# rhofield/rho-tts

Measured on AMD Instinct MI355X. Metric: audio-sec/wall-sec (RTF) Qwen3-TTS-1.7B batch=32, higher is better.
Workload: dtype bf16; 1 GPU; Qwen3-TTS-1.7B bf16, batch 32/GPU, 30-s reference clone, 10-word sentences (44 frames each), sampling=top-k 50 T 0.9, seeded synthetic weights; value counts delivered (post-processed) audio; global_batch=32, parallelism=dp1

## Files before the change

rho_tts_amd/csrc/generate.hip:

```cpp
#include "model_internal.h"

using namespace rtm;

namespace {

__global__ void k_frame_inc(int32_t* f) { if (threadIdx.x == 0) *f += 1; }
}

struct rt_gen_run {
    struct Staging { std::vector<int32_t> tid, cid, slot, pos, last, dst; };
    struct Lane {
        int b0 = 0, n = 0;
        hipStream_t stream = nullptr;
        float *xt = nullptr, *hn_f32 = nullptr, *xp = nullptr, *logits = nullptr, *rowsq_t = nullptr, *rowsq_p = nullptr;
        bf16_t *hn = nullptr, *hn_p = nullptr;
        int32_t *d_slot_b = nullptr, *d_pos_b = nullptr, *d_pos_p2 = nullptr, *d_zero_pos = nullptr, *d_frame = nullptr, *d_frame_off = nullptr;
        int64_t* d_items = nullptr;
        uint8_t* d_seen = nullptr;
        DecWs dwt, dwp;
        StackWs wt, wp;
        bool done = false;
    };
    rt_model* m = nullptr;
    rt_ctx* ctx = nullptr;
// ... 375 lines not shown
            ns = 1;
        } else {
            RT_TRY(gemm_rows(m, ln.hn_p + roff * Hp, n, PW(m, "pred.head" + std::to_string(q)), ln.logits, &ns));
        }
        SampleArgs sp{};
        sp.logits = ln.logits; sp.n_slabs = ns; sp.M = n; sp.V = Vp;
        sp.do_sample = A.predictor.do_sample; sp.temperature = A.predictor.temperature; sp.top_k = A.predictor.top_k;
        sp.top_p = A.predictor.top_p; sp.rep_penalty = 1.0f; sp.seen = nullptr; sp.suppress_from = Vp; sp.allow_token = -1;
        sp.seed_ptr = d_seed; sp.item_ids = ln.d_items; sp.frame = 0; sp.group = q + 1;
        sp.forced = d_forced ? d_forced + (size_t)(q + 1) * B + ln.b0 : nullptr; sp.forced_fs = (int64_t)G * B;
        sp.out = codes + q + 1; sp.out_stride = G; sp.out_fs = codes_fs; sp.eos_token = -1; sp.eos_flag = nullptr; sp.eos_fs = 0;
        sp.logits_copy = A.d_trace_predictor ? A.d_trace_predictor + ((size_t)q * B + ln.b0) * Vp : nullptr;
        sp.copy_fs = (int64_t)(G - 1) * B * Vp;
        sp.frame_ptr = ln.d_frame; sp.frame_off = ln.d_frame_off; sp.eos_live = 0; sp.min_frames = 0;
        const bool fuse_emb = col && m->has_mtp() && g_fuse_sample_embed && q < G - 2 && Vp <= 4096 && Hp % 8 == 0;
        if (fuse_emb) {
            sp.emb_table = m->proj_emb[q]; sp.emb_H = Hp; sp.emb_norm_w = m->pred.L[0].ln1; sp.emb_rowsq = ln.rowsq_p; sp.emb_rowsq_n = NTp;
            sp.emb_x_tiled = ln.dwp.xT; sp.emb_a_tiled = ln.dwp.xa;
        }
        RT_TRY(launch_sample(ctx, sp));
        if (q < G - 2) {
            if (fuse_emb) {
            } else if (col && m->has_mtp()) {
                RT_TRY(launch_embed_rowsq(ctx, nullptr, 0, m->proj_emb[q], codes + q + 1, G, ln.d_frame, codes_fs, n, Hp, nullptr, ln.rowsq_p,
                                          NTp, ln.dwp.xT, ln.dwp.xa, m->pred.L[0].ln1));
            } else if (col) {
                RT_TRY(launch_embed_rowsq(ctx, m->d_frame_srcs + q + 1, 1, nullptr, codes + q + 1, G, ln.d_frame, codes_fs, n, Hp, nullptr,
                                          ln.rowsq_p, NTp, ln.dwp.xT, ln.dwp.xa, m->pred.L[0].ln1));
            } else if (m->has_mtp()) RT_TRY(launch_gather_f32(ctx, m->proj_emb[q], Hp, codes + q + 1, n, ln.xp, nullptr, G, ln.d_frame, codes_fs));
            else RT_TRY(launch_gather_sum(ctx, m->d_frame_srcs + q + 1, 1, codes + q + 1, n, H, nullptr, nullptr, nullptr, ln.xp, nullptr, G, ln.d_frame, codes_fs));
            m->prof_class = 2;
            if (col) {
                RT_TRY(stack_decode(m, m->pred, ln.dwp, ln.dwp.xT, ln.rowsq_p, n, ln.d_slot_b, ln.d_zero_pos, q + 2, true, nullptr, ln.b0, true));
            } else {
                RT_TRY(stack_forward(m, m->pred, ln.wp, ln.xp, n, ln.d_slot_b, ln.d_zero_pos, q + 2, ln.hn_p, nullptr));
            }
        }
    }
    m->prof_class = 0;
    return RT_OK;
}

int rt_gen_run::enqueue_b(Lane& ln) {
    const int n = ln.n;
    int32_t* codes = d_codes + (size_t)ln.b0 * G;
    const bool inc_early = col && G <= 16 && g_frame_inc_fold;
    if (col && G <= 16) {
        RT_TRY(launch_embed_rowsq(ctx, m->d_frame_srcs, G, nullptr, codes, G, ln.d_frame, codes_fs, n, H, pad_t, ln.rowsq_t, NTt, ln.dwt.xT,
// ... 275 lines not shown
```

rho_tts_amd/csrc/kernels.h:

```cpp
#pragma once
#include "common.h"
#include "knobs.h"

struct PackedW {
    const bf16_t* data = nullptr;
    int N = 0, K = 0;
    int Np = 0, Kp = 0;
    size_t bytes() const { return (size_t)Np * Kp * 2; }
    const bf16_t* data16 = nullptr;
    int Np16 = 0;
};

struct GemmA {
    const void* ptr = nullptr;
    const void* ptr_lo = nullptr;
    int is_f32 = 0;
    int split = 0;
    int64_t M = 0;
    int Cin = 0;
    int taps = 1;
    int tap_stride = 1;
    int tap_offset = 0;
    int rows_out = 0;
    int rows_in = 0;
// ... 67 lines not shown
int launch_gemm_col(rt_ctx* ctx, const ColArgs& a, const PackedW& w, hipEvent_t ev_start = nullptr, hipEvent_t ev_stop = nullptr);
struct RowsqGather {
    const float* table = nullptr;
    const int32_t* idx = nullptr;
    int idx_stride = 1, first = 0;
    const int32_t* frame_ptr = nullptr;
    int64_t idx_frame_stride = 0;
};
int launch_rowsq(rt_ctx* ctx, const float* x, int M, int H, float* rowsq, int rowsq_n, float* x_tiled = nullptr,
                 bf16_t* a_tiled = nullptr, const float* norm_w = nullptr, const int32_t* src_rows = nullptr,
                 const int32_t* dst_rows = nullptr, const RowsqGather* gather = nullptr);

struct GatherSrc;
int launch_embed_rowsq(rt_ctx* ctx, const GatherSrc* d_srcs, int n_src, const float* f32_table, const int32_t* d_idx, int idx_stride,
                       const int32_t* frame_ptr, int64_t idx_frame_stride, int M, int H, const float* add_vec, float* rowsq, int rowsq_n,
                       float* x_tiled, bf16_t* a_tiled, const float* norm_w, int32_t* frame_inc = nullptr, unsigned* arrive = nullptr);

int launch_norm_tiled_rows(rt_ctx* ctx, const float* x_tiled, const float* rowsq, int rowsq_n, const float* w, float eps, int M, int H,
                           float* out);

int launch_add_rmsnorm(rt_ctx* ctx, float* x, int M, int H, const float* slabs, int n_slabs, const float* slab_bias,
                       const float* scale, const float* w, float eps, bf16_t* out_bf16, float* out_f32);
int launch_silu_mul(rt_ctx* ctx, const float* slabs, int n_slabs, int M, int I, bf16_t* out, float* out_f32 = nullptr);
int launch_reduce_slabs(rt_ctx* ctx, const float* slabs, int n_slabs, int64_t M, int N, const float* bias, int act,
                        float* out_f32, bf16_t* out_bf16);

struct KvCache {
    bf16_t* k = nullptr;
    bf16_t* v = nullptr;
    int layers = 0, slots = 0, kv_heads = 0, max_pos = 0, head_dim = 0;
    bf16_t* k_lo = nullptr;
// ... 66 lines not shown
    int eos_token;
    int32_t* eos_flag;
    float* logits_copy;
    const int32_t* frame_ptr;
    const int32_t* frame_off;
    int64_t out_fs, eos_fs, forced_fs, copy_fs;
    int eos_live, min_frames;
    long long* stamps;
    const float* emb_table;
    int emb_H;
    const float* emb_norm_w;
    float* emb_rowsq;
    int emb_rowsq_n;
    float* emb_x_tiled;
    bf16_t* emb_a_tiled;
};
int launch_sample(rt_ctx* ctx, const SampleArgs& a);


int launch_dwconv_ln(rt_ctx* ctx, const float* x, int B, int T, int C, const float* w , const float* b,
                     const float* ln_w, const float* ln_b, float eps, float* out_f32);
int launch_code_embed_mean(rt_ctx* ctx, const bf16_t* table, int codebook, int Q, int H, const int32_t* codes ,
                           int64_t rows, float* out_f32);

bool launch_final_conv_ok(int C);
int launch_final_conv(rt_ctx* ctx, const bf16_t* hi, const bf16_t* lo, int B, int T, int C, const float* w, const float* bias, float* wav,
                      int64_t wav_stride);
int launch_f32_to_bf16(rt_ctx* ctx, const float* x, int64_t n, bf16_t* out);

int launch_enc_conv0(rt_ctx* ctx, const float* pcm, int64_t T, int C, int k, const float* w , const float* bias, float* x,
// ... 5 lines not shown
```

rho_tts_amd/csrc/knobs.h:

```cpp
#pragma once
#include "common.h"

#define RT_KNOBS(X) \
    X(0, g_skinny_variant, 0, 0, 2, "legacy skinny GEMM: 0 k_gemm_skinny, 1 k_gemm_skinny2<.,4>, 2 k_gemm_skinny2<.,8>") \
    X(100, g_decode_col, 1, 0, 1, "0 legacy 9-launch split-K decode, 1 column-owner GEMM + fused attention (5 launches per layer)") \
    X(200, g_use_graph, 1, 0, 1, "0 eager decode frames, 1 replayed from captured hipGraphs") \
    X(300, g_pred_nt, 0, 0, 1, "predictor weights: 0 cacheable loads (Infinity-Cache resident across its 15 passes), 1 non-temporal") \
    X(400, g_decode_lanes, 1, 1, 8, "decode lanes: groups of items decoding concurrently on their own streams (rt_generate)") \
    X(500, g_col_split, 0, 0, 4, "sub-tile split of narrow decode GEMMs: 0 automatic (col_split_for), 1 / 2 / 4 forced") \
    X(600, g_tile96, 1, 0, 1, "1: 128x96 workgroup tiles for N = 96 / 192 (codec decoder), 0: always 128x128") \
    X(700, g_col_rows64, 1, 0, 1, "1: one 64-row decode GEMM launch for the predictor's two-position pass, 0: two 32-row launches") \
    X(800, g_fuse_sample_embed, 1, 0, 1, "1: sampler + next-input embedding in one launch (predictor groups), 0: separate k_embed_rowsq") \
    X(900, g_prefill_fill, 3, 0, 99, "workgroups per CU a prefill GEMM's split-K aims for") \
    X(1000, g_xcd_order, 1, 0, 1, "1: tiled GEMMs run a row tile's column tiles back to back on one XCD") \
    X(1100, g_final_conv, 1, 0, 1, "the codec decoder's last conv: 1 its own LDS-window kernel, 0 a one-column GEMM") \
    X(1200, g_conv_win, 1, 0, 1, "1: k>1 convs on operand planes keep their input window in LDS (k_conv_win), 0: per-tap kernel") \
    X(1300, g_sync_parts, 0, 0, 1, "1: rt_generate waits for the stream after every frame part (bounds the dispatches in flight; profiling aid)") \
    X(1400, g_eos_check_every, 8, 1, 99, "frames between two host looks at the device-side end-of-sequence flags (1 = every frame)") \
    X(1500, g_attn_mfma, 0, 0, 2, "the talker's shared-prefix decode attention: 0 vector unit, 1 / 2 matrix cores with four rows / one row per workgroup (attention_mfma.hip); 1 measured " \
        "16.6 us per launch against 13.3 us for the vector-unit kernel at batch 32 / 460 prefix rows, so off") \
    X(1600, g_col_split4, 0, 0, 1, "1: the automatic split may go to quarter tiles (N <= 1024 on 256 CUs); measured 1.4 ms/step slower than half tiles") \
    X(1700, g_handover_every, 4, 1, 99, "queued items (n_items > rows): frames between two looks at the flags + row hand-overs.  Measured on the 1.7B model, 512 / 64 ragged texts on 32 " \
        "rows: 2 -> 487 / 445, 3 -> 489 / 445, 4 -> 491 / 447, 6 -> 485 / 445, 8 -> 477 / 428, 12 -> 475 / 434 audio-s/s (a hand-over costs ~1.4 ms, a waiting row 0.13 ms per frame)") \
    X(1800, g_conv_tall, 1, 0, 2, "k>1 convs of the 96- / 192-channel stages: 0 128-row tiles, 1 256-row tiles for long inputs, 2 always") \
    X(1900, g_prefill_mid, 1, 0, 3, "prompt prefills of 65..1024 rows: 0 split-K tiled kernel, 1 k_gemm_mid (no split-K slabs), 2 / 3 force its 64 / 128 tiles") \
    X(2000, g_col_max_rows, 64, 1, 64, "batches up to this many rows decode on the column-owner path.  Above 32 the talker's GEMMs take 64 rows per launch and the predictor's " \
        "two-position first pass runs as two 64-row launches: 715 audio-s/s at batch 64 against 510 at batch 32 (1.7B, bench.py --batch 64) - every weight byte serves twice the rows for " \
        "~1.4x the launch time") \
    X(2100, g_fuse_conv, 1, 0, 1, "1: a 96-channel k>1 conv and the 1x1 conv behind its activation run as one launch (launch_conv_pair); 0 switches the 192-channel pairs off as well") \
    X(2200, g_prefill_attn_mfma, 1, 0, 1, "prompt attention behind a shared voice prefix: 0 vector unit, 1 matrix cores") \
    X(2300, g_col_rows16, 0, 0, 1, "1: decode GEMM launches of <= 16 rows take the 128-VGPR MT = 1 instantiation (two workgroups per CU: decode lanes)") \
    X(2400, g_col_silu_x, 1, 0, 1, "1: gate/up GEMMs whose pairs are 1.5x the CUs run as one round of 1.5-pair workgroups, 0: one pair per workgroup (1.5 rounds)") \
    X(2600, g_conv_unroll, 1, 0, 1, "1: k = 7 convs run the tap-unrolled instantiation of k_conv_win, 0: the generic tap loop") \
    X(2700, g_frame_inc_fold, 0, 0, 1, "1: frame += 1 by the last workgroup of the frame's talker-input launch, 0: k_frame_inc (the fold measured 1-1.8 ms per step SLOWER)") \
    X(2800, g_pair_attn, 1, 0, 1, "1: two-position decode passes append both positions inside the fused attention launch, 0: k_qkv_post + k_attention") \
    X(2900, g_c2w_lean, 1, 0, 1, "1: rt_code2wav drops the third unit's unread residual-stream store and the waveform copy (the last conv writes the caller's buffer)") \
    X(3000, g_fuse_conv192, 1, 0, 1, "1: the 192-channel conv pairs fuse as well, weight fragments staged through LDS")

#define RT_KNOB_ARG(X) \
    X(0, g_skinny_waves_per_cu, 4, 1, 0x7fffffff, "legacy skinny GEMM: split-K is chosen so that about this many waves per CU stream weights")

#define RT_KNOB_EXTERN(base, name, def, lo, hi, doc) extern rt_knob name;
RT_KNOBS(RT_KNOB_EXTERN)
RT_KNOB_ARG(RT_KNOB_EXTERN)
#undef RT_KNOB_EXTERN
extern std::atomic<int> g_tune_epoch;
```

rho_tts_amd/csrc/model_internal.h:

```cpp
#pragma once

#include <algorithm>
#include <chrono>
#include <map>
#include <memory>

#include "kernels.h"


enum SlotKind { K_GEMM = 0, K_TABLE = 1, K_VEC = 2 };

struct Slot {
    std::string name;
    int kind = 0;
    int64_t rows = 0, cols = 0;
    bool set = false;
    PackedW pw;
    bf16_t* tbl = nullptr;
    float* vec = nullptr;
    void* raw = nullptr;
    void* raw16 = nullptr;
};

struct LayerW {
// ... 24 lines not shown
    int64_t last_frames_run = 0, last_rows = 0, last_kept = 0, last_swaps = 0;
    double last_launch_host_us = 0.0;
    rt_ctx* ctx = nullptr;
    rt_model_config cfg{};
    std::vector<Slot> slots;
    std::map<std::string, int> by_name;
    bool finalized = false;
    StackW talker, pred, ctf, etf;
    std::vector<int> enc_ch;
    const float** d_cbT = nullptr;
    std::vector<int> dec_ch;
    float* pad_t = nullptr;
    int pad_t_id = -1;
    float* proj_c0 = nullptr;
    std::vector<float*> proj_emb;
    GatherSrc* d_frame_srcs = nullptr;
    std::vector<float*> exp_vecs;
    std::map<std::string, float*> xvec;
    int prefix_len = 0;
    std::vector<PoolBlock> pool;
    bool prof = false;
    std::vector<std::pair<hipEvent_t, hipEvent_t>> prof_ev;
    size_t prof_used = 0;
    double prof_bytes = 0;
    int prof_class = 0;
    std::vector<std::pair<uint8_t, double>> prof_tag;
    uint64_t graph_sig = 0;
    std::vector<hipGraphExec_t> graphs;
    std::vector<hipStream_t> lane_streams;
    std::vector<hipEvent_t> lane_events;
// ... 44 lines not shown
    bf16_t* act = nullptr;
    float* q = nullptr;
    float* xT = nullptr;
    bf16_t* xa = nullptr;
};
struct TextWs { bf16_t *e = nullptr, *h1 = nullptr; GatherSrc* d_src = nullptr; };
bool prof_events(rt_model* m, double bytes, hipEvent_t* a, hipEvent_t* b);
int gemm_rows(rt_model* m, const bf16_t* A, int rows, const PackedW& W, float* slabs, int* n_slabs);
int gemm_rows_f32(rt_model* m, const float* A, int rows, const PackedW& W, float* slabs, int* n_slabs);
size_t slab_floats(const rt_stack_dims& d, int M, int n_cu = 256);
int alloc_stack_ws(rt_model* m, const rt_stack_dims& d, int M, StackWs* w, bool precise = false);
int stack_forward(rt_model* m, StackW& S, StackWs& w, float* x, int M, const int32_t* row_slot, const int32_t* row_pos, int pos_add,
                  bf16_t* out_bf16, float* out_f32, const int32_t* frame_ptr = nullptr, bool prefix_rows = false);
int alloc_dec_ws(rt_model* m, const rt_stack_dims& d, int M, DecWs* w);
int col_gemm(rt_model* m, const ColArgs& a0, const PackedW& W, bool is_predictor = false);
int stack_decode(rt_model* m, StackW& S, DecWs& w, float* x, float* rowsq, int M, const int32_t* row_slot, const int32_t* row_pos,
                 int pos_add, bool one_row_per_slot = true, const int32_t* frame_ptr = nullptr, int slot_base = -1, bool zero_pos = false);
int col_head(rt_model* m, const bf16_t* xa, const float* rowsq, int rowsq_n, int row_off, int M, int K, float eps,
             const PackedW& W, const float* bias, float* out);
int alloc_text_ws(rt_model* m, int n, TextWs* w);
int text_project(rt_model* m, const int32_t* d_ids, int n, float* out, const TextWs* ws = nullptr);

}
```

rho_tts_amd/csrc/model_load.hip:

```cpp
#include "model_internal.h"

namespace {

__global__ void k_bf16_to_f32(const bf16_t* __restrict__ x, int64_t n, float* __restrict__ out) {
    for (int64_t i = (int64_t)blockIdx.x * blockDim.x + threadIdx.x; i < n; i += (int64_t)gridDim.x * blockDim.x) out[i] = bf16_to_f32(x[i]);
}
__global__ void k_fill_i32(int32_t* p, int n, int v, int step_every, int step) {
    for (int i = blockIdx.x * blockDim.x + threadIdx.x; i < n; i += gridDim.x * blockDim.x) p[i] = v + (step_every > 0 ? (i / step_every) * step : 0);
}
}

namespace rtm {

int pool_get(rt_model* m, size_t bytes, void** out) {
    if (bytes == 0) bytes = 16;
    int best = -1;
    for (size_t i = 0; i < m->pool.size(); ++i)
        if (!m->pool[i].used && m->pool[i].size >= bytes && (best < 0 || m->pool[i].size < m->pool[best].size)) best = (int)i;
    if (best >= 0 && m->pool[best].size <= bytes * 2 + (1 << 20)) {
        m->pool[best].used = true;
        m->pool[best].tag = m->pool_tag;
        *out = m->pool[best].p;
        return RT_OK;
    }
// ... 171 lines not shown
        RT_HIP(m->ctx, hipMemsetAsync(S.kv.v_lo, 0, bytes, m->ctx->stream));
    }
    return RT_OK;
}

int expand_vec(rt_model* m, const float* src, int n, int reps, float** out) {
    float* p = nullptr;
    RT_HIP(m->ctx, hipMalloc((void**)&p, (size_t)n * reps * sizeof(float)));
    for (int r = 0; r < reps; ++r)
        RT_HIP(m->ctx, hipMemcpyAsync(p + (size_t)r * n, src, (size_t)n * sizeof(float), hipMemcpyDeviceToDevice, m->ctx->stream));
    m->exp_vecs.push_back(p);
    *out = p;
    return RT_OK;
}

}

extern "C" {

int rt_model_create(rt_ctx* ctx, const rt_model_config* cfg, rt_model** out_model) {
    if (!ctx || !cfg || !out_model) return rt_fail(ctx, RT_ERR_INVALID, "rt_model_create: null argument");
    *out_model = nullptr;
    const rt_model_config& c = *cfg;
    auto bad_stack = [](const rt_stack_dims& d) {
        return d.hidden < 16 || d.hidden % 16 || d.layers < 1 || d.heads < 1 || d.kv_heads < 1 || d.heads % d.kv_heads ||
               (d.head_dim != 32 && d.head_dim != 64 && d.head_dim != 128) || d.inter % 16 || (d.heads * d.head_dim) % 32 ||
               (d.kv_heads * d.head_dim) % 16;
    };
    if (bad_stack(c.talker) || bad_stack(c.predictor) || bad_stack(c.codec_tf))
        return rt_fail(ctx, RT_ERR_INVALID, "rt_model_create: unsupported stack dimensions (hidden/inter %% 16, head_dim in {32,64,128})");
// ... 29 lines not shown
    for (auto& s : m->slots) { if (s.raw) (void)hipFree(s.raw); if (s.raw16) (void)hipFree(s.raw16); }
    if (m->d_cbT) (void)hipFree((void*)m->d_cbT);
    for (StackW* S : {&m->talker, &m->pred, &m->ctf, &m->etf}) {
        if (S->kv.k) (void)hipFree(S->kv.k);
        if (S->kv.v) (void)hipFree(S->kv.v);
        if (S->kv.k_lo) (void)hipFree(S->kv.k_lo);
        if (S->kv.v_lo) (void)hipFree(S->kv.v_lo);
        if (S->kv.vt_prefix) (void)hipFree(S->kv.vt_prefix);
        if (S->kv.kt_prefix) (void)hipFree(S->kv.kt_prefix);
        if (S->cos) (void)hipFree(S->cos);
        if (S->sin) (void)hipFree(S->sin);
    }
    for (auto& b : m->pool) (void)hipFree(b.p);
    for (auto p : m->exp_vecs) (void)hipFree(p);
    for (auto p : m->proj_emb) (void)hipFree(p);
    if (m->proj_c0) (void)hipFree(m->proj_c0);
    if (m->pad_t) (void)hipFree(m->pad_t);
    if (m->d_frame_srcs) (void)hipFree(m->d_frame_srcs);
    for (auto& e : m->prof_ev) { (void)hipEventDestroy(e.first); (void)hipEventDestroy(e.second); }
    for (auto ex : m->graphs) if (ex) (void)hipGraphExecDestroy(ex);
    for (auto st : m->lane_streams) { (void)hipStreamSynchronize(st); (void)hipStreamDestroy(st); }
    for (auto ev : m->lane_events) (void)hipEventDestroy(ev);
    if (m->fork_event) (void)hipEventDestroy(m->fork_event);
    delete m;
    return RT_OK;
}

int rt_model_tensor_count(rt_model* m) { return m ? (int)m->slots.size() : -1; }

int rt_model_tensor_info(rt_model* m, int32_t index, char* name, size_t name_cap, int64_t* shape2, int32_t* kind) {
// ... 108 lines not shown
    for (int gq = 1; gq < c.n_groups; ++gq) srcs[gq] = {TBL(m, "pred.emb" + std::to_string(gq - 1)), c.talker.hidden};
    RT_HIP(ctx, hipMalloc((void**)&m->d_frame_srcs, sizeof(GatherSrc) * c.n_groups));
    RT_HIP(ctx, hipMemcpy(m->d_frame_srcs, srcs.data(), sizeof(GatherSrc) * c.n_groups, hipMemcpyHostToDevice));
    if (m->has_mtp()) {
        const int Hp = c.predictor.hidden, H = c.talker.hidden;
        auto project = [&](const bf16_t* tbl, int rows, float** out) -> int {
            RT_HIP(ctx, hipMalloc((void**)out, (size_t)rows * Hp * 4));
            GemmA a; a.ptr = tbl; a.M = rows; a.Cin = H;
            GemmEpi e; e.bias = VEC(m, "pred.mtp_b"); e.out_f32 = *out; e.ldc = Hp;
            return launch_gemm(ctx, a, PW(m, "pred.mtp"), e);
        };
        RT_TRY(project(TBL(m, "talker.codec_embedding"), c.codec_vocab, &m->proj_c0));
        m->proj_emb.resize(c.n_groups - 1, nullptr);
        for (int gq = 0; gq < c.n_groups - 1; ++gq) RT_TRY(project(TBL(m, "pred.emb" + std::to_string(gq)), c.predictor_vocab, &m->proj_emb[gq]));
    }
    for (int i = 0; i < c.n_upsample_rates; ++i) {
        const std::string bn = "codec.b" + std::to_string(i);
        for (const char* v : {".u0.a1", ".u0.ib1"}) {
            float* x = nullptr;
            RT_TRY(expand_vec(m, VEC(m, bn + v), m->dec_ch[i + 1], c.upsample_rates[i], &x));
            m->xvec[bn + v] = x;
        }
    }
    RT_HIP(ctx, hipStreamSynchronize(ctx->stream));
    m->finalized = true;
    return RT_OK;
}

int64_t rt_model_weight_bytes(rt_model* m) { return m ? m->weight_bytes : -1; }

// ... 49 lines not shown
```

rho_tts_amd/csrc/model_stack.hip:

```cpp
#include "model_internal.h"

namespace rtm {

bool prof_events(rt_model* m, double bytes, hipEvent_t* a, hipEvent_t* b) {
    *a = *b = nullptr;
    if (!m->prof) return false;
    if (m->prof_used >= m->prof_ev.size()) {
        if (m->prof_ev.size() >= 400000) return false;
        hipEvent_t x, y;
        if (hipEventCreate(&x) != hipSuccess || hipEventCreate(&y) != hipSuccess) return false;
        m->prof_ev.push_back({x, y});
    }
    if (m->prof_tag.size() <= m->prof_used) m->prof_tag.resize(m->prof_used + 1);
    m->prof_tag[m->prof_used] = {(uint8_t)m->prof_class, bytes};
    auto& pr = m->prof_ev[m->prof_used++];
    *a = pr.first;
    *b = pr.second;
    m->prof_bytes += bytes;
    return true;
}

int gemm_rows(rt_model* m, const bf16_t* A, int rows, const PackedW& W, float* slabs, int* n_slabs) {
    if (rows <= 64) {
        const int S = skinny_pick_split(rows, W.N, W.K, m->ctx->n_cu);
// ... 122 lines not shown
    return RT_OK;
}
int col_gemm(rt_model* m, const ColArgs& a0, const PackedW& W, bool is_predictor) {
    const int blk = g_col_rows64 ? 64 : 32;
    for (int r0 = 0; r0 < a0.M; r0 += blk) {
        ColArgs a = a0;
        a.nt = is_predictor ? g_pred_nt.load() : 1;
        a.M = std::min(blk, a0.M - r0);
        a.row_off = a0.row_off + r0;
        hipEvent_t e0, e1;
        prof_events(m, (double)W.N * W.K * 2.0, &e0, &e1);
        RT_TRY(launch_gemm_col(m->ctx, a, W, e0, e1));
    }
    return RT_OK;
}
int stack_decode(rt_model* m, StackW& S, DecWs& w, float* x, float* rowsq, int M, const int32_t* row_slot, const int32_t* row_pos,
                 int pos_add, bool one_row_per_slot, const int32_t* frame_ptr, int slot_base, bool zero_pos) {
    rt_ctx* ctx = m->ctx;
    const rt_stack_dims& d = S.d;
    const int H = d.hidden, sp_h = col_split_for(H, ctx->n_cu), NTh = H / 16 * sp_h, qw = (d.heads + 2 * d.kv_heads) * d.head_dim;
    const bool isp = &S == &m->pred;
    for (int i = 0; i < d.layers; ++i) {
        LayerW& L = S.L[i];
        const float* next_w = (i + 1 < d.layers) ? S.L[i + 1].ln1 : S.norm;
        ColArgs a;
        a.A = w.xa; a.post_scale = 1; a.rowsq = rowsq; a.rowsq_n = NTh; a.eps = d.rms_eps; a.M = M; a.K = H;
        a.epi = COL_STORE; a.out = w.qkv; a.ldc = qw; a.split = col_split_for(qw, ctx->n_cu);
        RT_TRY(col_gemm(m, a, L.wqkv, isp));
        if (one_row_per_slot) {
            RT_TRY(launch_attention_fused(ctx, w.qkv, M, d.heads, d.kv_heads, d.head_dim, L.qn, L.kn, d.rms_eps, S.cos, S.sin, slot_base >= 0 ? nullptr : row_slot,
                                          zero_pos ? nullptr : row_pos, pos_add, S.window, S.kv, i, w.ao, frame_ptr, 1, slot_base));
        } else if (g_pair_attn && M % 2 == 0 && d.heads <= 2 * d.kv_heads && d.heads % d.kv_heads == 0 && row_slot && row_pos) {
            RT_TRY(launch_attention_fused(ctx, w.qkv, M, d.heads, d.kv_heads, d.head_dim, L.qn, L.kn, d.rms_eps, S.cos, S.sin, row_slot, row_pos, pos_add,
                                          S.window, S.kv, i, w.ao, frame_ptr, 1, -1, M / 2));
        } else {
            RT_TRY(launch_qkv_post(ctx, w.qkv, 1, M, d.heads, d.kv_heads, d.head_dim, L.qn, L.kn, d.rms_eps, S.cos, S.sin, row_slot, row_pos,
                                   pos_add, w.q, S.kv, i, frame_ptr));
            RT_TRY(launch_attention(ctx, w.q, M, d.heads, d.kv_heads, d.head_dim, row_slot, row_pos, pos_add, S.window, S.kv, i, w.ao, frame_ptr, 1));
        }
        ColArgs o;
        o.A = w.ao; o.M = M; o.K = d.heads * d.head_dim; o.epi = COL_RESID; o.out = x; o.ldc = H; o.scale = L.ls1;
        o.rowsq_out = rowsq; o.rowsq_out_n = NTh; o.next_bf16 = w.xa; o.next_norm_w = L.ln2; o.split = sp_h;
        RT_TRY(col_gemm(m, o, L.wo, isp));
// ... 47 lines not shown
```

rho_tts_amd/csrc/rowops.hip:

```cpp
#include "kernels.h"

namespace {

typedef __attribute__((ext_vector_type(4))) float f4_t;

__device__ __forceinline__ float block_sum_f32(float v, float* sh) {
    v = wave_sum_f32(v);
    const int w = threadIdx.x >> 6, nw = (blockDim.x + 63) >> 6;
    __syncthreads();
    if ((threadIdx.x & 63) == 0) sh[w] = v;
    __syncthreads();
    float t = 0.f;
    for (int i = 0; i < nw; ++i) t += sh[i];
    return t;
}

__global__ __launch_bounds__(256) void k_add_rmsnorm(float* __restrict__ x, int H, const float* __restrict__ slabs, int n_slabs,
                                                     int64_t slab_stride, const float* __restrict__ slab_bias,
                                                     const float* __restrict__ scale, const float* __restrict__ w, float eps,
                                                     bf16_t* __restrict__ out_bf16, float* __restrict__ out_f32) {
    __shared__ float sh[4];
    constexpr int MAXV = 8;
    const int64_t row = blockIdx.x;
    const int nv = H >> 2;
// ... 132 lines not shown
            uint2 pk;
            pk.x = f32x2_to_bf16x2(wv[0] * v[0], wv[1] * v[1]);
            pk.y = f32x2_to_bf16x2(wv[2] * v[2], wv[3] * v[3]);
            *reinterpret_cast<uint2*>(a_tiled + tile_off((int)row, i * 4, H)) = pk;
        }
    }
    const float tot = block_sum_f32(ss, sh);
    for (int j = threadIdx.x; j < rowsq_n; j += 256) rowsq[row * rowsq_n + j] = j == 0 ? tot : 0.f;
}

__global__ __launch_bounds__(256) void k_embed_rowsq(const GatherSrc* __restrict__ srcs, int n_src, const float* __restrict__ f32_table,
                                                     const int32_t* __restrict__ idx, int idx_stride,
                                                     const int32_t* __restrict__ frame_ptr, int64_t idx_frame_stride, int H,
                                                     const float* __restrict__ add_vec, float* __restrict__ rowsq, int rowsq_n,
                                                     float* __restrict__ x_tiled, bf16_t* __restrict__ a_tiled,
                                                     const float* __restrict__ norm_w, int32_t* frame_inc, unsigned* arrive) {
    constexpr int MAXS = 16;
    __shared__ const bf16_t* sh_tab[MAXS];
    __shared__ float sh[4];
    const int row = blockIdx.x, tid = threadIdx.x;
    if (frame_ptr) idx += (int64_t)(frame_inc ? __atomic_load_n(frame_ptr, __ATOMIC_RELAXED) : *frame_ptr) * idx_frame_stride;
    if (tid < MAXS) {
        const bf16_t* p = nullptr;
        if (tid < n_src) {
            const int id = idx[(int64_t)row * idx_stride + tid];
            if (id >= 0) p = srcs[tid].table + (int64_t)id * srcs[tid].row_stride;
        }
        sh_tab[tid] = p;
    }
    const int fid = f32_table ? idx[(int64_t)row * idx_stride] : -1;
    __syncthreads();
    if (frame_inc && tid == 0 && atomicAdd(arrive, 1u) == gridDim.x - 1) {
        *arrive = 0u;
        atomicAdd(frame_inc, 1);
    }
    float ss = 0.f;
    for (int c = tid * 8; c < H; c += 2048) {
        uint4 raw[MAXS];
#pragma unroll
        for (int j = 0; j < MAXS; ++j) {
            const bf16_t* p = sh_tab[j];
            raw[j] = p ? *reinterpret_cast<const uint4*>(p + c) : uint4{0u, 0u, 0u, 0u};
        }
        float v[8];
#pragma unroll
// ... 15 lines not shown
                }
            }
        }
#pragma unroll
        for (int e = 0; e < 8; ++e) ss += v[e] * v[e];
        const int64_t o = tile_off(row, c, H);
        *reinterpret_cast<f4_t*>(x_tiled + o) = f4_t{v[0], v[1], v[2], v[3]};
        *reinterpret_cast<f4_t*>(x_tiled + o + 4) = f4_t{v[4], v[5], v[6], v[7]};
        const f4_t w0 = *reinterpret_cast<const f4_t*>(norm_w + c), w1 = *reinterpret_cast<const f4_t*>(norm_w + c + 4);
        uint4 pk;
        pk.x = f32x2_to_bf16x2(w0[0] * v[0], w0[1] * v[1]);
        pk.y = f32x2_to_bf16x2(w0[2] * v[2], w0[3] * v[3]);
        pk.z = f32x2_to_bf16x2(w1[0] * v[4], w1[1] * v[5]);
        pk.w = f32x2_to_bf16x2(w1[2] * v[6], w1[3] * v[7]);
        *reinterpret_cast<uint4*>(a_tiled + o) = pk;
    }
    const float tot = block_sum_f32(ss, sh);
    for (int j = tid; j < rowsq_n; j += 256) rowsq[(int64_t)row * rowsq_n + j] = j == 0 ? tot : 0.f;
}

__global__ __launch_bounds__(256) void k_norm_tiled_rows(const float* __restrict__ x_tiled, const float* __restrict__ rowsq, int rowsq_n,
                                                         const float* __restrict__ w, float eps, int H, float* __restrict__ out) {
    __shared__ float sh[4];
    const int row = blockIdx.x;
    float s = 0.f;
    for (int j = threadIdx.x; j < rowsq_n; j += 256) s += rowsq[(int64_t)row * rowsq_n + j];
    const float inv = rsqrtf(block_sum_f32(s, sh) / (float)H + eps);
    for (int c = threadIdx.x * 4; c < H; c += 1024) {
        const f4_t v = *reinterpret_cast<const f4_t*>(x_tiled + tile_off(row, c, H));
        const f4_t wv = *reinterpret_cast<const f4_t*>(w + c);
// ... 251 lines not shown
}

int launch_rowsq(rt_ctx* ctx, const float* x, int M, int H, float* rowsq, int rowsq_n, float* x_tiled, bf16_t* a_tiled,
                 const float* norm_w, const int32_t* src_rows, const int32_t* dst_rows, const RowsqGather* gather) {
    if (M <= 0) return RT_OK;
    const RowsqGather gt = gather ? *gather : RowsqGather{};
    if (gt.table && (src_rows || dst_rows || gt.first < 0 || gt.first > M || !gt.idx))
        return rt_fail(ctx, RT_ERR_INVALID, "rowsq: gathered rows take no row maps (first %d of %d rows)", gt.first, M);
    hipLaunchKernelGGL(k_rowsq, dim3(M), dim3(256), 0, ctx->stream, x, H, rowsq, rowsq_n, x_tiled, a_tiled, norm_w, src_rows, dst_rows, gt);
    RT_HIP(ctx, hipGetLastError());
    return RT_OK;
}

int launch_embed_rowsq(rt_ctx* ctx, const GatherSrc* d_srcs, int n_src, const float* f32_table, const int32_t* d_idx, int idx_stride,
                       const int32_t* frame_ptr, int64_t idx_frame_stride, int M, int H, const float* add_vec, float* rowsq, int rowsq_n,
                       float* x_tiled, bf16_t* a_tiled, const float* norm_w, int32_t* frame_inc, unsigned* arrive) {
    if (M <= 0) return RT_OK;
    if (n_src > 16 || H % 8 || !x_tiled || !a_tiled || !norm_w || !rowsq || rowsq_n < 1 || (n_src > 0 && !d_srcs))
        return rt_fail(ctx, RT_ERR_INVALID, "embed_rowsq: n_src %d (<= 16), H %d (multiple of 8) or a missing buffer", n_src, H);
    if (frame_inc && (f32_table || !arrive || frame_inc != frame_ptr))
        return rt_fail(ctx, RT_ERR_INVALID, "embed_rowsq: the frame counter is advanced by launches over bf16 sources only, with an arrival counter");
    hipLaunchKernelGGL(k_embed_rowsq, dim3(M), dim3(256), 0, ctx->stream, d_srcs, n_src, f32_table, d_idx, idx_stride, frame_ptr,
                       idx_frame_stride, H, add_vec, rowsq, rowsq_n, x_tiled, a_tiled, norm_w, frame_inc, arrive);
    RT_HIP(ctx, hipGetLastError());
    return RT_OK;
}

int launch_norm_tiled_rows(rt_ctx* ctx, const float* x_tiled, const float* rowsq, int rowsq_n, const float* w, float eps, int M, int H,
                           float* out) {
    if (M <= 0) return RT_OK;
    if (H % 8) return rt_fail(ctx, RT_ERR_INVALID, "norm_tiled_rows: H %d not a multiple of 8", H);
    hipLaunchKernelGGL(k_norm_tiled_rows, dim3(M), dim3(256), 0, ctx->stream, x_tiled, rowsq, rowsq_n, w, eps, H, out);
    RT_HIP(ctx, hipGetLastError());
    return RT_OK;
}

int launch_silu_mul(rt_ctx* ctx, const float* slabs, int n_slabs, int M, int I, bf16_t* out, float* out_f32) {
    const int64_t total = (int64_t)M * I / 4;
// ... 88 lines not shown
```

rho_tts_amd/csrc/sampling.hip:

```cpp
#include "kernels.h"

namespace {

__device__ __forceinline__ unsigned mix32(unsigned h) {
    h ^= h >> 16; h *= 0x85EBCA6Bu; h ^= h >> 13; h *= 0xC2B2AE35u; h ^= h >> 16;
    return h;
}
__device__ __forceinline__ float rt_uniform(uint64_t seed, unsigned item, unsigned frame, unsigned group) {
    const unsigned a = mix32((unsigned)(seed & 0xffffffffu) ^ 0x85EBCA6Bu);
    const unsigned b = mix32(a + item * 0x9E3779B1u);
    const unsigned c = mix32(b + frame * 0x85EBCA77u);
    const unsigned d = mix32(c + group * 0xC2B2AE3Du + (unsigned)(seed >> 32));
    return __fmul_rn(__fadd_rn((float)(d >> 8), 0.5f), 1.0f / 16777216.0f);
}
__device__ __forceinline__ unsigned okey(float f) {
    const unsigned u = __float_as_uint(f);
    return (u & 0x80000000u) ? ~u : (u | 0x80000000u);
}

struct Cand { float v; int idx; };
__device__ __forceinline__ bool before(const Cand& a, const Cand& b) { return a.v > b.v || (a.v == b.v && a.idx < b.idx); }

__global__ __launch_bounds__(256) void k_sample(SampleArgs A) {
    extern __shared__ float vals[];
// ... 466 lines not shown
        __syncthreads();
    }
    if (A.stamps && row == 0 && tid == 0) A.stamps[6] = wall_clock64();
    if (tid == 0) {
        if (seen && token >= 0 && token < V) seen[token] = 1;
        int is_eos = 0;
        if (A.eos_token >= 0 && token == A.eos_token) { is_eos = 1; token = 0; }
        if (A.eos_flag) A.eos_flag[row] = is_eos;
        A.out[(int64_t)row * A.out_stride] = token;
        sh_i[0] = token;
    }
    if (A.emb_table) {
        __syncthreads();
        const int tok = sh_i[0];
        const int H = A.emb_H;
        float ss = 0.f;
        if (tid < 256) {
            for (int c = tid * 8; c < H; c += 2048) {
                float e[8];
                const f4s_t a = *reinterpret_cast<const f4s_t*>(A.emb_table + (int64_t)tok * H + c);
                const f4s_t b = *reinterpret_cast<const f4s_t*>(A.emb_table + (int64_t)tok * H + c + 4);
#pragma unroll
                for (int q = 0; q < 4; ++q) { e[q] = 0.f + a[q]; e[4 + q] = 0.f + b[q]; }
#pragma unroll
                for (int q = 0; q < 8; ++q) ss += e[q] * e[q];
                const int64_t o = tile_off(row, c, H);
                *reinterpret_cast<f4s_t*>(A.emb_x_tiled + o) = f4s_t{e[0], e[1], e[2], e[3]};
                *reinterpret_cast<f4s_t*>(A.emb_x_tiled + o + 4) = f4s_t{e[4], e[5], e[6], e[7]};
                const f4s_t w0 = *reinterpret_cast<const f4s_t*>(A.emb_norm_w + c), w1 = *reinterpret_cast<const f4s_t*>(A.emb_norm_w + c + 4);
                uint4 pk;
// ... 10 lines not shown
        __syncthreads();
        const float tot = ((sh_f[0] + sh_f[1]) + sh_f[2]) + sh_f[3];
        for (int j = tid; j < A.emb_rowsq_n; j += NT) A.emb_rowsq[(int64_t)row * A.emb_rowsq_n + j] = j == 0 ? tot : 0.f;
    }
}

}

int launch_sample(rt_ctx* ctx, const SampleArgs& a) {
    if (a.M <= 0) return RT_OK;
    if (a.do_sample && (a.top_k < 1 || a.top_k > 64)) return rt_fail(ctx, RT_ERR_INVALID, "sampling needs 1 <= top_k <= 64 (got %d)", a.top_k);
    if (a.do_sample && !(a.temperature > 0.f)) return rt_fail(ctx, RT_ERR_INVALID, "sampling needs temperature > 0");
    if (a.V > 16384) return rt_fail(ctx, RT_ERR_UNSUPPORTED, "vocabulary %d too large for the sampler", a.V);
    if (a.emb_table && (a.V > 4096 || a.emb_H % 8 || !a.emb_norm_w || !a.emb_rowsq || a.emb_rowsq_n < 1 || !a.emb_x_tiled || !a.emb_a_tiled))
        return rt_fail(ctx, RT_ERR_INVALID, "sample: fused embedding needs V <= 4096, H %% 8 == 0 and all its buffers");
    if (a.V <= 1024) hipLaunchKernelGGL((k_sample_w<4, 4>), dim3(a.M), dim3(256), 0, ctx->stream, a);
    else if (a.V <= 2048) hipLaunchKernelGGL((k_sample_w<4, 8>), dim3(a.M), dim3(512), 0, ctx->stream, a);
    else if (a.V <= 4096) hipLaunchKernelGGL((k_sample_w<4, 16>), dim3(a.M), dim3(1024), 0, ctx->stream, a);
    else hipLaunchKernelGGL(k_sample, dim3(a.M), dim3(256), a.V * sizeof(float), ctx->stream, a);
    RT_HIP(ctx, hipGetLastError());
    return RT_OK;
}
```

Before: 569.7 audio-s/s.

## Precompute predictor layer-0 QKV per code and copy rows instead of GEMM

At model load, the predictor's layer-0 q/k/v projection is precomputed for every code in each codebook group, giving per-group tables of vocab by qkv-width floats. During decode, the kernel that embeds the drawn code (fused sampler or embed_rowsq) also copies that code's qkv row into the workspace, and stack_decode skips the layer-0 QKV GEMM. This removes one GEMM launch and its weight streaming per predictor pass. In exchange it costs extra load time and memory for the tables, adds per-row copy traffic, and the fused sampler path no longer writes the normalized bf16 activations or rowsq, which is safe only if layer 0 never reads them.

```diff
diff --git a/rho_tts_amd/csrc/generate.hip b/rho_tts_amd/csrc/generate.hip
--- a/rho_tts_amd/csrc/generate.hip
+++ b/rho_tts_amd/csrc/generate.hip
@@ -413,24 +413,27 @@
         sp.copy_fs = (int64_t)(G - 1) * B * Vp;
         sp.frame_ptr = ln.d_frame; sp.frame_off = ln.d_frame_off; sp.eos_live = 0; sp.min_frames = 0;
         const bool fuse_emb = col && m->has_mtp() && g_fuse_sample_embed && q < G - 2 && Vp <= 4096 && Hp % 8 == 0;
+        const float* qkv_tab = (col && g_pred_qkv_table && q < G - 2 && q < (int)m->pred_qkv0.size()) ? m->pred_qkv0[q] : nullptr;
+        const int qw_p = (c.predictor.heads + 2 * c.predictor.kv_heads) * c.predictor.head_dim;
         if (fuse_emb) {
             sp.emb_table = m->proj_emb[q]; sp.emb_H = Hp; sp.emb_norm_w = m->pred.L[0].ln1; sp.emb_rowsq = ln.rowsq_p; sp.emb_rowsq_n = NTp;
             sp.emb_x_tiled = ln.dwp.xT; sp.emb_a_tiled = ln.dwp.xa;
+            sp.emb_qkv_table = qkv_tab; sp.emb_qkv_out = ln.dwp.qkv; sp.emb_qkv_n = qw_p;
         }
         RT_TRY(launch_sample(ctx, sp));
         if (q < G - 2) {
             if (fuse_emb) {
             } else if (col && m->has_mtp()) {
                 RT_TRY(launch_embed_rowsq(ctx, nullptr, 0, m->proj_emb[q], codes + q + 1, G, ln.d_frame, codes_fs, n, Hp, nullptr, ln.rowsq_p,
-                                          NTp, ln.dwp.xT, ln.dwp.xa, m->pred.L[0].ln1));
+                                          NTp, ln.dwp.xT, ln.dwp.xa, m->pred.L[0].ln1, nullptr, nullptr, qkv_tab, ln.dwp.qkv, qw_p));
             } else if (col) {
                 RT_TRY(launch_embed_rowsq(ctx, m->d_frame_srcs + q + 1, 1, nullptr, codes + q + 1, G, ln.d_frame, codes_fs, n, Hp, nullptr,
-                                          ln.rowsq_p, NTp, ln.dwp.xT, ln.dwp.xa, m->pred.L[0].ln1));
+                                          ln.rowsq_p, NTp, ln.dwp.xT, ln.dwp.xa, m->pred.L[0].ln1, nullptr, nullptr, qkv_tab, ln.dwp.qkv, qw_p));
             } else if (m->has_mtp()) RT_TRY(launch_gather_f32(ctx, m->proj_emb[q], Hp, codes + q + 1, n, ln.xp, nullptr, G, ln.d_frame, codes_fs));
             else RT_TRY(launch_gather_sum(ctx, m->d_frame_srcs + q + 1, 1, codes + q + 1, n, H, nullptr, nullptr, nullptr, ln.xp, nullptr, G, ln.d_frame, codes_fs));
             m->prof_class = 2;
             if (col) {
-                RT_TRY(stack_decode(m, m->pred, ln.dwp, ln.dwp.xT, ln.rowsq_p, n, ln.d_slot_b, ln.d_zero_pos, q + 2, true, nullptr, ln.b0, true));
+                RT_TRY(stack_decode(m, m->pred, ln.dwp, ln.dwp.xT, ln.rowsq_p, n, ln.d_slot_b, ln.d_zero_pos, q + 2, true, nullptr, ln.b0, true, qkv_tab != nullptr));
             } else {
                 RT_TRY(stack_forward(m, m->pred, ln.wp, ln.xp, n, ln.d_slot_b, ln.d_zero_pos, q + 2, ln.hn_p, nullptr));
             }
diff --git a/rho_tts_amd/csrc/kernels.h b/rho_tts_amd/csrc/kernels.h
--- a/rho_tts_amd/csrc/kernels.h
+++ b/rho_tts_amd/csrc/kernels.h
@@ -105,7 +105,8 @@
 struct GatherSrc;
 int launch_embed_rowsq(rt_ctx* ctx, const GatherSrc* d_srcs, int n_src, const float* f32_table, const int32_t* d_idx, int idx_stride,
                        const int32_t* frame_ptr, int64_t idx_frame_stride, int M, int H, const float* add_vec, float* rowsq, int rowsq_n,
-                       float* x_tiled, bf16_t* a_tiled, const float* norm_w, int32_t* frame_inc = nullptr, unsigned* arrive = nullptr);
+                       float* x_tiled, bf16_t* a_tiled, const float* norm_w, int32_t* frame_inc = nullptr, unsigned* arrive = nullptr,
+                       const float* qkv_table = nullptr, float* qkv_out = nullptr, int qkv_n = 0);
 
 int launch_norm_tiled_rows(rt_ctx* ctx, const float* x_tiled, const float* rowsq, int rowsq_n, const float* w, float eps, int M, int H,
                            float* out);
@@ -202,6 +203,9 @@
     int emb_rowsq_n;
     float* emb_x_tiled;
     bf16_t* emb_a_tiled;
+    const float* emb_qkv_table;
+    float* emb_qkv_out;
+    int emb_qkv_n;
 };
 int launch_sample(rt_ctx* ctx, const SampleArgs& a);
 
diff --git a/rho_tts_amd/csrc/knobs.h b/rho_tts_amd/csrc/knobs.h
--- a/rho_tts_amd/csrc/knobs.h
+++ b/rho_tts_amd/csrc/knobs.h
@@ -35,7 +35,9 @@
     X(2700, g_frame_inc_fold, 0, 0, 1, "1: frame += 1 by the last workgroup of the frame's talker-input launch, 0: k_frame_inc (the fold measured 1-1.8 ms per step SLOWER)") \
     X(2800, g_pair_attn, 1, 0, 1, "1: two-position decode passes append both positions inside the fused attention launch, 0: k_qkv_post + k_attention") \
     X(2900, g_c2w_lean, 1, 0, 1, "1: rt_code2wav drops the third unit's unread residual-stream store and the waveform copy (the last conv writes the caller's buffer)") \
-    X(3000, g_fuse_conv192, 1, 0, 1, "1: the 192-channel conv pairs fuse as well, weight fragments staged through LDS")
+    X(3000, g_fuse_conv192, 1, 0, 1, "1: the 192-channel conv pairs fuse as well, weight fragments staged through LDS") \
+    X(3100, g_pred_qkv_table, 1, 0, 1, "predictor passes 2..G-1: 1 layer 0's q/k/v row of the drawn code is copied from the table rt_model_finalize builds (by the launch " \
+        "that embeds the code), 0 the layer-0 qkv GEMM launch runs (same bits either way)")
 
 #define RT_KNOB_ARG(X) \
     X(0, g_skinny_waves_per_cu, 4, 1, 0x7fffffff, "legacy skinny GEMM: split-K is chosen so that about this many waves per CU stream weights")
diff --git a/rho_tts_amd/csrc/model_internal.h b/rho_tts_amd/csrc/model_internal.h
--- a/rho_tts_amd/csrc/model_internal.h
+++ b/rho_tts_amd/csrc/model_internal.h
@@ -62,6 +62,7 @@
     int pad_t_id = -1;
     float* proj_c0 = nullptr;
     std::vector<float*> proj_emb;
+    std::vector<float*> pred_qkv0;
     GatherSrc* d_frame_srcs = nullptr;
     std::vector<float*> exp_vecs;
     std::map<std::string, float*> xvec;
@@ -136,8 +137,10 @@
                   bf16_t* out_bf16, float* out_f32, const int32_t* frame_ptr = nullptr, bool prefix_rows = false);
 int alloc_dec_ws(rt_model* m, const rt_stack_dims& d, int M, DecWs* w);
 int col_gemm(rt_model* m, const ColArgs& a0, const PackedW& W, bool is_predictor = false);
+int stack_qkv(rt_model* m, StackW& S, int layer, const bf16_t* xa, const float* rowsq, int M, float* out);
 int stack_decode(rt_model* m, StackW& S, DecWs& w, float* x, float* rowsq, int M, const int32_t* row_slot, const int32_t* row_pos,
-                 int pos_add, bool one_row_per_slot = true, const int32_t* frame_ptr = nullptr, int slot_base = -1, bool zero_pos = false);
+                 int pos_add, bool one_row_per_slot = true, const int32_t* frame_ptr = nullptr, int slot_base = -1, bool zero_pos = false,
+                 bool qkv0_ready = false);
 int col_head(rt_model* m, const bf16_t* xa, const float* rowsq, int rowsq_n, int row_off, int M, int K, float eps,
              const PackedW& W, const float* bias, float* out);
 int alloc_text_ws(rt_model* m, int n, TextWs* w);
diff --git a/rho_tts_amd/csrc/model_load.hip b/rho_tts_amd/csrc/model_load.hip
--- a/rho_tts_amd/csrc/model_load.hip
+++ b/rho_tts_amd/csrc/model_load.hip
@@ -209,6 +209,51 @@
     return RT_OK;
 }
 
+int build_pred_qkv0(rt_model* m) {
+    rt_ctx* ctx = m->ctx;
+    const rt_model_config& c = m->cfg;
+    const rt_stack_dims& d = c.predictor;
+    const int G = c.n_groups, Hp = d.hidden, Vp = c.predictor_vocab, qw = (d.heads + 2 * d.kv_heads) * d.head_dim;
+    if (G < 3 || Vp < 1 || Hp % 32 || d.inter % 32 || c.talker.hidden % 32 || c.talker.inter % 32 || qw % 4 || !m->pred.L[0].wqkv.data16) return RT_OK;
+    const int NTp = Hp / 16 * col_split_for(Hp, ctx->n_cu);
+    const size_t table_bytes = (size_t)Vp * qw * sizeof(float);
+    m->pred_qkv0.assign(G - 2, nullptr);
+    for (int q = 0; q < G - 2; ++q)
+        if (hipMalloc((void**)&m->pred_qkv0[q], table_bytes) != hipSuccess) {
+            (void)hipGetLastError();
+            for (auto p : m->pred_qkv0) if (p) (void)hipFree(p);
+            m->pred_qkv0.clear();
+            fprintf(stderr, "rho_tts_amd: no memory for the predictor's layer-0 q/k/v tables (%d x %.1f MB): their GEMM launches stay (same results)\n",
+                    G - 2, table_bytes / 1e6);
+            return RT_OK;
+        }
+    struct Tmp {
+        float *xT = nullptr, *rowsq = nullptr;
+        bf16_t* xa = nullptr;
+        int32_t* idx = nullptr;
+        ~Tmp() { (void)hipFree(xT); (void)hipFree(rowsq); (void)hipFree(xa); (void)hipFree(idx); }
+    } t;
+    RT_HIP(ctx, hipMalloc((void**)&t.xT, (size_t)32 * Hp * sizeof(float)));
+    RT_HIP(ctx, hipMalloc((void**)&t.xa, (size_t)32 * Hp * sizeof(bf16_t)));
+    RT_HIP(ctx, hipMalloc((void**)&t.rowsq, (size_t)32 * NTp * sizeof(float)));
+    RT_HIP(ctx, hipMalloc((void**)&t.idx, (size_t)Vp * sizeof(int32_t)));
+    RT_HIP(ctx, hipMemsetAsync(t.xT, 0, (size_t)32 * Hp * sizeof(float), ctx->stream));
+    RT_HIP(ctx, hipMemsetAsync(t.xa, 0, (size_t)32 * Hp * sizeof(bf16_t), ctx->stream));
+    RT_HIP(ctx, hipMemsetAsync(t.rowsq, 0, (size_t)32 * NTp * sizeof(float), ctx->stream));
+    int rc = launch_fill_i32(ctx, t.idx, Vp, 0, 1, 1);
+    for (int q = 0; q < G - 2 && !rc; ++q)
+        for (int c0 = 0; c0 < Vp && !rc; c0 += 32) {
+            const int nb = std::min(32, Vp - c0);
+            if (m->has_mtp()) rc = launch_embed_rowsq(ctx, nullptr, 0, m->proj_emb[q], t.idx + c0, 1, nullptr, 0, nb, Hp, nullptr, t.rowsq, NTp, t.xT, t.xa, m->pred.L[0].ln1);
+            else rc = launch_embed_rowsq(ctx, m->d_frame_srcs + q + 1, 1, nullptr, t.idx + c0, 1, nullptr, 0, nb, Hp, nullptr, t.rowsq, NTp, t.xT, t.xa, m->pred.L[0].ln1);
+            if (!rc) rc = stack_qkv(m, m->pred, 0, t.xa, t.rowsq, nb, m->pred_qkv0[q] + (size_t)c0 * qw);
+        }
+    const hipError_t se = hipStreamSynchronize(ctx->stream);
+    if (rc) return rc;
+    RT_HIP(ctx, se);
+    return RT_OK;
+}
+
 }
 
 extern "C" {
@@ -268,6 +313,7 @@
     for (auto& b : m->pool) (void)hipFree(b.p);
     for (auto p : m->exp_vecs) (void)hipFree(p);
     for (auto p : m->proj_emb) (void)hipFree(p);
+    for (auto p : m->pred_qkv0) (void)hipFree(p);
     if (m->proj_c0) (void)hipFree(m->proj_c0);
     if (m->pad_t) (void)hipFree(m->pad_t);
     if (m->d_frame_srcs) (void)hipFree(m->d_frame_srcs);
@@ -406,6 +452,7 @@
         m->proj_emb.resize(c.n_groups - 1, nullptr);
         for (int gq = 0; gq < c.n_groups - 1; ++gq) RT_TRY(project(TBL(m, "pred.emb" + std::to_string(gq)), c.predictor_vocab, &m->proj_emb[gq]));
     }
+    RT_TRY(build_pred_qkv0(m));
     for (int i = 0; i < c.n_upsample_rates; ++i) {
         const std::string bn = "codec.b" + std::to_string(i);
         for (const char* v : {".u0.a1", ".u0.ib1"}) {
diff --git a/rho_tts_amd/csrc/model_stack.hip b/rho_tts_amd/csrc/model_stack.hip
--- a/rho_tts_amd/csrc/model_stack.hip
+++ b/rho_tts_amd/csrc/model_stack.hip
@@ -160,19 +160,24 @@
     }
     return RT_OK;
 }
+int stack_qkv(rt_model* m, StackW& S, int layer, const bf16_t* xa, const float* rowsq, int M, float* out) {
+    const rt_stack_dims& d = S.d;
+    const int H = d.hidden, n_cu = m->ctx->n_cu, qw = (d.heads + 2 * d.kv_heads) * d.head_dim;
+    ColArgs a;
+    a.A = xa; a.post_scale = 1; a.rowsq = rowsq; a.rowsq_n = H / 16 * col_split_for(H, n_cu); a.eps = d.rms_eps; a.M = M; a.K = H;
+    a.epi = COL_STORE; a.out = out; a.ldc = qw; a.split = col_split_for(qw, n_cu);
+    return col_gemm(m, a, S.L[layer].wqkv, &S == &m->pred);
+}
 int stack_decode(rt_model* m, StackW& S, DecWs& w, float* x, float* rowsq, int M, const int32_t* row_slot, const int32_t* row_pos,
-                 int pos_add, bool one_row_per_slot, const int32_t* frame_ptr, int slot_base, bool zero_pos) {
+                 int pos_add, bool one_row_per_slot, const int32_t* frame_ptr, int slot_base, bool zero_pos, bool qkv0_ready) {
     rt_ctx* ctx = m->ctx;
     const rt_stack_dims& d = S.d;
-    const int H = d.hidden, sp_h = col_split_for(H, ctx->n_cu), NTh = H / 16 * sp_h, qw = (d.heads + 2 * d.kv_heads) * d.head_dim;
+    const int H = d.hidden, sp_h = col_split_for(H, ctx->n_cu), NTh = H / 16 * sp_h;
     const bool isp = &S == &m->pred;
     for (int i = 0; i < d.layers; ++i) {
         LayerW& L = S.L[i];
         const float* next_w = (i + 1 < d.layers) ? S.L[i + 1].ln1 : S.norm;
-        ColArgs a;
-        a.A = w.xa; a.post_scale = 1; a.rowsq = rowsq; a.rowsq_n = NTh; a.eps = d.rms_eps; a.M = M; a.K = H;
-        a.epi = COL_STORE; a.out = w.qkv; a.ldc = qw; a.split = col_split_for(qw, ctx->n_cu);
-        RT_TRY(col_gemm(m, a, L.wqkv, isp));
+        if (i > 0 || !qkv0_ready) RT_TRY(stack_qkv(m, S, i, w.xa, rowsq, M, w.qkv));
         if (one_row_per_slot) {
             RT_TRY(launch_attention_fused(ctx, w.qkv, M, d.heads, d.kv_heads, d.head_dim, L.qn, L.kn, d.rms_eps, S.cos, S.sin, slot_base >= 0 ? nullptr : row_slot,
                                           zero_pos ? nullptr : row_pos, pos_add, S.window, S.kv, i, w.ao, frame_ptr, 1, slot_base));
diff --git a/rho_tts_amd/csrc/rowops.hip b/rho_tts_amd/csrc/rowops.hip
--- a/rho_tts_amd/csrc/rowops.hip
+++ b/rho_tts_amd/csrc/rowops.hip
@@ -170,7 +170,8 @@
                                                      const int32_t* __restrict__ frame_ptr, int64_t idx_frame_stride, int H,
                                                      const float* __restrict__ add_vec, float* __restrict__ rowsq, int rowsq_n,
                                                      float* __restrict__ x_tiled, bf16_t* __restrict__ a_tiled,
-                                                     const float* __restrict__ norm_w, int32_t* frame_inc, unsigned* arrive) {
+                                                     const float* __restrict__ norm_w, int32_t* frame_inc, unsigned* arrive,
+                                                     const float* __restrict__ qkv_table, float* __restrict__ qkv_out, int qkv_n) {
     constexpr int MAXS = 16;
     __shared__ const bf16_t* sh_tab[MAXS];
     __shared__ float sh[4];
@@ -185,6 +186,19 @@
         sh_tab[tid] = p;
     }
     const int fid = f32_table ? idx[(int64_t)row * idx_stride] : -1;
+    constexpr int QU = 4;
+    const int n4 = qkv_n >> 2;
+    f4_t qv[QU];
+    const f4_t* qsrc = nullptr;
+    if (qkv_table) {
+        const int qid = idx[(int64_t)row * idx_stride];
+        qsrc = reinterpret_cast<const f4_t*>(qkv_table + (int64_t)(qid < 0 ? 0 : qid) * qkv_n);
+#pragma unroll
+        for (int u = 0; u < QU; ++u) {
+            const int i = tid + u * 256;
+            qv[u] = qsrc[i < n4 ? i : n4 - 1];
+        }
+    }
     __syncthreads();
     if (frame_inc && tid == 0 && atomicAdd(arrive, 1u) == gridDim.x - 1) {
         *arrive = 0u;
@@ -230,6 +244,15 @@
         pk.z = f32x2_to_bf16x2(w1[0] * v[4], w1[1] * v[5]);
         pk.w = f32x2_to_bf16x2(w1[2] * v[6], w1[3] * v[7]);
         *reinterpret_cast<uint4*>(a_tiled + o) = pk;
+    }
+    if (qkv_table) {
+        f4_t* qdst = reinterpret_cast<f4_t*>(qkv_out + (int64_t)row * qkv_n);
+#pragma unroll
+        for (int u = 0; u < QU; ++u) {
+            const int i = tid + u * 256;
+            if (i < n4) qdst[i] = qv[u];
+        }
+        for (int i = tid + QU * 256; i < n4; i += 256) qdst[i] = qsrc[i];
     }
     const float tot = block_sum_f32(ss, sh);
     for (int j = tid; j < rowsq_n; j += 256) rowsq[(int64_t)row * rowsq_n + j] = j == 0 ? tot : 0.f;
@@ -511,14 +534,17 @@
 
 int launch_embed_rowsq(rt_ctx* ctx, const GatherSrc* d_srcs, int n_src, const float* f32_table, const int32_t* d_idx, int idx_stride,
                        const int32_t* frame_ptr, int64_t idx_frame_stride, int M, int H, const float* add_vec, float* rowsq, int rowsq_n,
-                       float* x_tiled, bf16_t* a_tiled, const float* norm_w, int32_t* frame_inc, unsigned* arrive) {
+                       float* x_tiled, bf16_t* a_tiled, const float* norm_w, int32_t* frame_inc, unsigned* arrive, const float* qkv_table,
+                       float* qkv_out, int qkv_n) {
     if (M <= 0) return RT_OK;
     if (n_src > 16 || H % 8 || !x_tiled || !a_tiled || !norm_w || !rowsq || rowsq_n < 1 || (n_src > 0 && !d_srcs))
         return rt_fail(ctx, RT_ERR_INVALID, "embed_rowsq: n_src %d (<= 16), H %d (multiple of 8) or a missing buffer", n_src, H);
     if (frame_inc && (f32_table || !arrive || frame_inc != frame_ptr))
         return rt_fail(ctx, RT_ERR_INVALID, "embed_rowsq: the frame counter is advanced by launches over bf16 sources only, with an arrival counter");
+    if (qkv_table && (!qkv_out || qkv_n < 4 || qkv_n % 4 || frame_inc || (f32_table ? n_src != 0 : n_src != 1)))
+        return rt_fail(ctx, RT_ERR_INVALID, "embed_rowsq: the q/k/v table takes one code per row, an output and a row width that is a multiple of 4");
     hipLaunchKernelGGL(k_embed_rowsq, dim3(M), dim3(256), 0, ctx->stream, d_srcs, n_src, f32_table, d_idx, idx_stride, frame_ptr,
-                       idx_frame_stride, H, add_vec, rowsq, rowsq_n, x_tiled, a_tiled, norm_w, frame_inc, arrive);
+                       idx_frame_stride, H, add_vec, rowsq, rowsq_n, x_tiled, a_tiled, norm_w, frame_inc, arrive, qkv_table, qkv_out, qkv_n);
     RT_HIP(ctx, hipGetLastError());
     return RT_OK;
 }
diff --git a/rho_tts_amd/csrc/sampling.hip b/rho_tts_amd/csrc/sampling.hip
--- a/rho_tts_amd/csrc/sampling.hip
+++ b/rho_tts_amd/csrc/sampling.hip
@@ -504,6 +504,39 @@
         __syncthreads();
         const int tok = sh_i[0];
         const int H = A.emb_H;
+        if (A.emb_qkv_table) {
+            constexpr int QU = 2;
+            const int n4 = A.emb_qkv_n >> 2, H8 = H >> 3;
+            const f4s_t* __restrict__ qsrc = reinterpret_cast<const f4s_t*>(A.emb_qkv_table + (int64_t)tok * A.emb_qkv_n);
+            f4s_t* __restrict__ qdst = reinterpret_cast<f4s_t*>(A.emb_qkv_out + (int64_t)row * A.emb_qkv_n);
+            const float* __restrict__ esrc = A.emb_table + (int64_t)tok * H;
+            const int e0 = tid < H8 ? tid : H8 - 1;
+            const f4s_t ea = *reinterpret_cast<const f4s_t*>(esrc + e0 * 8), eb = *reinterpret_cast<const f4s_t*>(esrc + e0 * 8 + 4);
+            f4s_t qv[QU];
+#pragma unroll
+            for (int u = 0; u < QU; ++u) {
+                const int i = tid + u * NT;
+                qv[u] = qsrc[i < n4 ? i : n4 - 1];
+            }
+            if (tid < H8) {
+                const int64_t o = tile_off(row, tid * 8, H);
+                *reinterpret_cast<f4s_t*>(A.emb_x_tiled + o) = f4s_t{0.f + ea[0], 0.f + ea[1], 0.f + ea[2], 0.f + ea[3]};
+                *reinterpret_cast<f4s_t*>(A.emb_x_tiled + o + 4) = f4s_t{0.f + eb[0], 0.f + eb[1], 0.f + eb[2], 0.f + eb[3]};
+            }
+#pragma unroll
+            for (int u = 0; u < QU; ++u) {
+                const int i = tid + u * NT;
+                if (i < n4) qdst[i] = qv[u];
+            }
+            for (int e = tid + NT; e < H8; e += NT) {
+                const f4s_t a = *reinterpret_cast<const f4s_t*>(esrc + e * 8), b = *reinterpret_cast<const f4s_t*>(esrc + e * 8 + 4);
+                const int64_t o = tile_off(row, e * 8, H);
+                *reinterpret_cast<f4s_t*>(A.emb_x_tiled + o) = f4s_t{0.f + a[0], 0.f + a[1], 0.f + a[2], 0.f + a[3]};
+                *reinterpret_cast<f4s_t*>(A.emb_x_tiled + o + 4) = f4s_t{0.f + b[0], 0.f + b[1], 0.f + b[2], 0.f + b[3]};
+            }
+            for (int i = tid + QU * NT; i < n4; i += NT) qdst[i] = qsrc[i];
+            return;
+        }
         float ss = 0.f;
         if (tid < 256) {
             for (int c = tid * 8; c < H; c += 2048) {
@@ -544,6 +577,8 @@
     if (a.V > 16384) return rt_fail(ctx, RT_ERR_UNSUPPORTED, "vocabulary %d too large for the sampler", a.V);
     if (a.emb_table && (a.V > 4096 || a.emb_H % 8 || !a.emb_norm_w || !a.emb_rowsq || a.emb_rowsq_n < 1 || !a.emb_x_tiled || !a.emb_a_tiled))
         return rt_fail(ctx, RT_ERR_INVALID, "sample: fused embedding needs V <= 4096, H %% 8 == 0 and all its buffers");
+    if (a.emb_qkv_table && (!a.emb_table || !a.emb_qkv_out || a.emb_qkv_n < 4 || a.emb_qkv_n % 4))
+        return rt_fail(ctx, RT_ERR_INVALID, "sample: the q/k/v table needs the fused embedding, an output and a row width that is a multiple of 4");
     if (a.V <= 1024) hipLaunchKernelGGL((k_sample_w<4, 4>), dim3(a.M), dim3(256), 0, ctx->stream, a);
     else if (a.V <= 2048) hipLaunchKernelGGL((k_sample_w<4, 8>), dim3(a.M), dim3(512), 0, ctx->stream, a);
     else if (a.V <= 4096) hipLaunchKernelGGL((k_sample_w<4, 16>), dim3(a.M), dim3(1024), 0, ctx->stream, a);
```

Result: faster. 576.8 audio-s/s, median of 6 (+1.2%).
